# DiltheyLab/MetaMaps

Hardware: AMD Instinct MI355X
Metric: Gbp long reads mapped+classified per sec (whole node), miniSeq+H DB (higher is better)
Workload: dtype u32

## Files before the change

metamaps_amd/csrc/mm_l1.hpp:

```cpp
#pragma once
#include <rocprim/rocprim.hpp>
#include "mm_map.hpp"
#include "mm_l2.hpp"

namespace mm {

template <int IPT>
__global__ void __launch_bounds__(256) sort_hits_radix_kernel(uint64_t* __restrict__ hits, const uint64_t* __restrict__ read_hit_off,
                                                              const int32_t* __restrict__ read_list, int end_bit,
                                                              const uint64_t* __restrict__ stage ,
                                                              const uint64_t* __restrict__ stage_off ) {
  using Sort = rocprim::block_radix_sort<uint64_t, 256, IPT>;
  extern __shared__ __align__(16) unsigned char sort_dyn[];
  typename Sort::storage_type& tmp = *reinterpret_cast<typename Sort::storage_type*>(sort_dyn);
  const int r = read_list[blockIdx.x];
  const uint64_t o = read_hit_off[r];
  const int n = (int)(read_hit_off[r + 1] - o);
  const uint64_t* __restrict__ src = hits + o;
  if (stage) { const uint64_t sb = stage_off[r]; if ((uint64_t)n <= stage_off[r + 1] - sb) src = stage + sb; }
  uint64_t key[IPT];
#pragma unroll
  for (int i = 0; i < IPT; ++i) { const int idx = threadIdx.x * IPT + i; key[i] = idx < n ? src[idx] : ~0ull; }
  Sort().sort(key, tmp, 0, end_bit);
#pragma unroll
  for (int i = 0; i < IPT; ++i) { const int idx = threadIdx.x * IPT + i; if (idx < n) hits[o + idx] = key[i]; }
}

template <bool WRITE>
__global__ void l1_scan_kernel(const uint64_t* __restrict__ hits, const uint64_t* __restrict__ read_hit_off, const int32_t* __restrict__ read_len,
                               const int32_t* __restrict__ min_hits, int64_t n_reads, uint32_t* __restrict__ cand_n,
                               const uint64_t* __restrict__ cand_off, int32_t* __restrict__ cand, int32_t* __restrict__ cand_read) {
  int64_t r = (int64_t)blockIdx.x * blockDim.x + threadIdx.x;
  if (r >= n_reads) return;
  const uint64_t o = read_hit_off[r];
  const int64_t H = (int64_t)(read_hit_off[r + 1] - o);
  const int len = read_len[r];
  int m = min_hits[r]; if (m < 1) m = 1;
  uint32_t nc = 0;
  int lseq = -1, lstart = 0, lend = 0;
  uint64_t wbase = WRITE ? cand_off[r] : 0;
  auto flush = [&]() {
    if (lseq < 0) return;
    if (WRITE) { int32_t* c = cand + 3 * (wbase + nc); c[0] = lseq; c[1] = lstart; c[2] = lend; cand_read[wbase + nc] = (int32_t)r; }
    ++nc;
  };
// ... 166 lines not shown
```

metamaps_amd/csrc/mm_map.hip:

```cpp
#include "mm_map.hpp"
#include <functional>
#include <memory>
#include <rocprim/rocprim.hpp>
#include "mm_l2_core.hpp"
#include "mm_size_classes.hpp"
#include "mm_l2.hpp"
#include "mm_l2z.hpp"
#include "mm_l2_dense.hpp"
#include <cstdlib>
#include <atomic>
#include <thread>
#include "mm_stats.hpp"
#include <algorithm>
#include <numeric>
#include "mm_sketch.hpp"
#include "mm_seed.hpp"
#include "mm_l1.hpp"

namespace mm {

namespace {
struct HostLap {
  const bool on = getenv("MM_HOST_TIMING") != nullptr; std::chrono::steady_clock::time_point t = std::chrono::steady_clock::now();
  void operator()(const char* what) { if (!on) return; const auto n = std::chrono::steady_clock::now(); fprintf(stderr, "host %-28s %8.1f us\n", what, std::chrono::duration<double, std::micro>(n - t).count()); t = n; }
// ... 161 lines not shown
  std::unique_ptr<SkipClasses> sk;

  MapRun(mm_ctx* ctx_, const mm_index* I_, const mm_seqset* reads_, const mm_map_params& P_, mm_mapping* M_)
      : ctx(ctx_), I(I_), reads(reads_), P(P_), M(M_), st(ctx_->stream), T(st), n(reads_->count()) {}

  const std::vector<uint64_t>& hoff() const { return M->mz.h_off; }
  int min_mapped_len() const { return P.w + P.k + 1; }
  bool dense_read(int64_t r, int sr) const { return sr >= sw.dense_from && sr < L2_SKETCH_LIMIT && M->read_len[(size_t)r] >= min_mapped_len(); }
  bool filtering() const { return sw.use_filter && n > 0; }

  void begin() {
    MM_REQUIRE(M->sketch_only || (I && I->k == P.k && I->w == P.w), MM_ERR_ARG, "index was built with different k / window size");
    MM_REQUIRE(n < (1LL << 31), MM_ERR_LIMIT, "more than 2^31 reads in one batch");
    M->ctx = ctx; M->n_reads = n; M->params = P; M->stats = mm_map_stats{};
    M->stats.n_reads = n;
    M->read_len = reads->len;
    M->active.assign((size_t)n, 0);
    for (int64_t r = 0; r < n; ++r) {
      int L = reads->len[(size_t)r];
      bool ok = !(L < P.w || L < P.k || L < P.min_read_len);
      M->active[(size_t)r] = ok;
      if (ok) { M->stats.n_reads_long_enough++; M->stats.bases_long_enough += L; }
    }
    t_total = T.begin(&M->stats.ms_total);
  }

  void minimizers() {
    const mm_mapping* const donor = M->sketch_donor;
    if (donor) {
      const size_t t = T.begin(&M->stats.ms_minimizer);
      auto dcopy = [&](auto& dst, const auto& src) { dst.alloc(src.n); if (src.n) MM_HIP(hipMemcpyAsync(dst.p, src.p, src.bytes(), hipMemcpyDeviceToDevice, st)); };
      mm_mapping* const dn = const_cast<mm_mapping*>(donor);
      const bool same_ctx = donor->ctx == ctx;
      if (same_ctx) M->mz.rec.share_from(dn->mz.rec); else dcopy(M->mz.rec, donor->mz.rec);
      dcopy(M->mz.off, donor->mz.off);
      M->mz.h_off = donor->mz.h_off; M->mz.total = donor->mz.total;
      if (same_ctx) M->sk_hash.share_from(dn->sk_hash); else dcopy(M->sk_hash, donor->sk_hash);
      dcopy(M->sk_strand, donor->sk_strand); dcopy(M->sk_n, donor->sk_n); dcopy(M->amb, donor->amb);
      T.end(t);
    } else { size_t t = T.begin(&M->stats.ms_minimizer); run_minimizers(ctx, reads, P.k, P.w, M->active, false, M->mz); T.end(t); }
    total_mz = M->mz.total;
    if (!donor) {
      M->sk_hash.alloc((size_t)std::max<int64_t>(total_mz, 1));
      M->sk_strand.alloc((size_t)std::max<int64_t>(total_mz, 1));
      M->sk_n.alloc((size_t)std::max<int64_t>(n, 1)); M->sk_n.zero(st);
      M->amb.alloc((size_t)std::max<int64_t>(n, 1)); M->amb.zero(st);
    }
  }

  void sketch() {
    if (M->sketch_donor) return;
    size_t t_sk = T.begin(&M->stats.ms_sketch);
    static_assert(ipt_list_is<4, 6, 8, 10, 12, 16, 20, 24, 32, 40, 48, 64>(SKETCH_IPTS), "the dispatch below lists the classes of mm_size_classes.hpp");
    uint64_t big_seen = 0;
    HostLap hl;
    const ReadBins RB = bin_reads(n, N_SKETCH_CLASSES, [&](int64_t r) -> int {
      const uint64_t c = hoff()[(size_t)r + 1] - hoff()[(size_t)r];
      big_seen |= (uint64_t)(c > SKETCH_LDS_MAX);
      return sketch_class_index(c);
    });
    const bool any_big = big_seen != 0;
    {
      hl("K2 bin");
      DBuf<int32_t> list(std::max<size_t>(RB.order.size(), 1));
      list.upload(RB.order.data(), RB.order.size(), st);
      hl("K2 list upload");
      size_t at = 0;
      for (auto& run : RB.runs) {
        const unsigned nb = (unsigned)run.second;
        const int32_t* lp = list.p + at;
        dispatch<4, 6, 8, 10, 12, 16, 20, 24, 32, 40, 48, 64>(SKETCH_IPTS[run.first], [&](auto ipt_tag) {
          constexpr int IPT = decltype(ipt_tag)::value;
          using SortT = rocprim::block_radix_sort<uint32_t, 256, IPT, uint16_t>;
          using ScanT = rocprim::block_scan<int, 256>;
          const size_t lds = std::max(sizeof(typename SortT::storage_type), sizeof(typename ScanT::storage_type)) + 16;
          if (lds > 48 * 1024) MM_HIP(hipFuncSetAttribute((const void*)sketch_radix_kernel<IPT>, hipFuncAttributeMaxDynamicSharedMemorySize, (int)lds));
          sketch_radix_kernel<IPT><<<dim3(nb), dim3(256), lds, st>>>(M->mz.rec.p, M->mz.off.p, lp, M->sk_hash.p, M->sk_strand.p, M->sk_n.p, M->amb.p);
        });
        MM_KERNEL_CHECK();
        at += run.second;
      }
      hl("K2 launches");
      MM_HIP(mm::stream_sync(st));
      hl("K2 sync (kernels)");
    }
    if (any_big) sketch_big_segmented();
    T.end(t_sk);
  }

  void sketch_big_segmented() {
    std::vector<int32_t> big; std::vector<uint64_t> koff{0};
    for (int64_t r = 0; r < n; ++r) { const uint64_t c = hoff()[(size_t)r + 1] - hoff()[(size_t)r]; if (c > SKETCH_LDS_MAX) { big.push_back((int32_t)r); koff.push_back(koff.back() + c); } }
    const size_t nb = big.size(); const uint64_t nk = koff.back();
    MM_REQUIRE(nk < ((uint64_t)1 << 32), MM_ERR_LIMIT, "more than 2^32 minimizers of reads beyond 16384 minimizers in one batch");
    DBuf<int32_t> d_big(nb); d_big.upload(big.data(), nb, st);
    DBuf<uint64_t> d_koff(nb + 1); d_koff.upload(koff.data(), nb + 1, st);
    DBuf<uint64_t> keys((size_t)nk), sorted((size_t)nk);
    sketch_keys_kernel<<<dim3((unsigned)nb), dim3(256), 0, st>>>(M->mz.rec.p, M->mz.off.p, d_big.p, d_koff.p, keys.p);
    MM_KERNEL_CHECK();
    size_t tmp_bytes = 0;
    MM_HIP(rocprim::segmented_radix_sort_keys(nullptr, tmp_bytes, keys.p, sorted.p, (unsigned int)nk, (unsigned int)nb, d_koff.p, d_koff.p + 1, 0, 64, st));
    DBuf<uint8_t> tmp(std::max<size_t>(tmp_bytes, 16));
    MM_HIP(rocprim::segmented_radix_sort_keys((void*)tmp.p, tmp_bytes, keys.p, sorted.p, (unsigned int)nk, (unsigned int)nb, d_koff.p, d_koff.p + 1, 0, 64, st));
    sketch_finish_kernel<<<dim3((unsigned)nb), dim3(256), 0, st>>>(M->mz.rec.p, M->mz.off.p, d_big.p, d_koff.p, sorted.p, M->sk_hash.p, M->sk_strand.p, M->sk_n.p, M->amb.p);
    MM_KERNEL_CHECK();
    MM_HIP(mm::stream_sync(st));
  }

  bool after_sketch() {
    hl.t = std::chrono::steady_clock::now();
    M->h_sk_n = M->sk_n.to_host(st, (size_t)n);
    if (M->sketch_only) {
      for (int64_t r = 0; r < n; ++r) M->stats.sum_sketch += M->h_sk_n[(size_t)r];
      M->h_rec_off.assign((size_t)n + 1, 0); M->n_rec = 0;
      T.end(t_total);
      T.collect();
      return false;
    }
    if (M->at_stage) M->at_stage(M->at_stage_user, 1);
    h_amb = M->amb.to_host(st, (size_t)n);
    hl("post-K2 downloads");
    int64_t giant = 0;
    for (int64_t r = 0; r < n; ++r) if (M->h_sk_n[(size_t)r] >= L2_SKETCH_LIMIT) ++giant;
    M->stats.n_reads_giant = giant;
    return true;
  }

  void tiebreak_lists() {
    for (int64_t r = 0; r < n; ++r) if (h_amb[(size_t)r]) (sw.eager_tiebreak ? eager_reads : lazy_reads).push_back(r);
    M->stats.n_ambiguous_sketch_reads = (int64_t)(eager_reads.size() + lazy_reads.size());
    hl("post-K2 amb lists");
    if (!eager_reads.empty()) amb_finish = start_tiebreak(eager_reads);
    hl("post-K2 tiebreak start");
  }

  std::function<void()> start_tiebreak(const std::vector<int64_t>& amb_reads) {
    const size_t na = amb_reads.size();
    std::vector<uint64_t> so(na), dof(na + 1, 0);
    std::vector<int32_t> expect(na);
    for (size_t i = 0; i < na; ++i) {
      int64_t r = amb_reads[i];
      so[i] = hoff()[(size_t)r];
      dof[i + 1] = dof[i] + (hoff()[(size_t)r + 1] - hoff()[(size_t)r]);
      expect[i] = M->h_sk_n[(size_t)r];
    }
    DBuf<uint64_t> d_so(na), d_do(na + 1);
    d_so.upload(so.data(), na, st); d_do.upload(dof.data(), na + 1, st);
    DBuf<Rec> comp((size_t)dof[na]);
    gather_amb_kernel<<<dim3((unsigned)na), dim3(256), 0, st>>>(M->mz.rec.p, d_so.p, d_do.p, comp.p);
    MM_KERNEL_CHECK();
    amb_states.push_back(std::make_unique<AmbState>());
    AmbState* const A = amb_states.back().get();
    A->hr = comp.to_host(st);
    A->dof = dof; A->expect = std::move(expect); A->d_so = std::move(d_so); A->d_do = std::move(d_do);
    A->sv.assign((size_t)dof[na], 0);
    A->scnt.assign(na, 0);
    A->bg = std::thread([A, na]() {
      std::atomic<size_t> next{0};
      auto worker = [&]() {
        std::vector<HostMz> v;
        for (size_t i = next.fetch_add(1); i < na; i = next.fetch_add(1)) {
          const size_t cntr = (size_t)(A->dof[i + 1] - A->dof[i]);
          v.resize(cntr);
          for (size_t j = 0; j < cntr; ++j) { const Rec& x = A->hr[(size_t)A->dof[i] + j]; v[j] = HostMz{x.hash, pw_wpos(x.pw), pw_strand(x.pw)}; }
          std::sort(v.begin(), v.end(), host_less_by_hash);
          auto ue = std::unique(v.begin(), v.end(), host_eq_by_hash);
          const size_t sN = (size_t)(ue - v.begin());
          if ((int64_t)sN != A->expect[i]) A->mismatch = 1;
          for (size_t j = 0; j < sN; ++j) A->sv[(size_t)A->dof[i] + j] = v[j].strand == 1 ? 1 : 0;
          A->scnt[i] = (int32_t)sN;
        }
      };
      const unsigned nthr = std::max(1u, std::min(32u, std::min<unsigned>(mm::cpu_budget(), (unsigned)((na + 15) / 16))));
      std::vector<std::thread> pool;
      for (unsigned t = 1; t < nthr; ++t) pool.emplace_back(worker);
      worker();
      for (auto& t : pool) t.join();
    });
    return [M = M, A, na, st = st]() {
      if (A->bg.joinable()) A->bg.join();
      MM_REQUIRE(A->mismatch == 0, MM_ERR_DEVICE, "sketch size disagrees between device and host tie-break");
      DBuf<uint8_t> d_sv(A->sv.size()); d_sv.upload(A->sv.data(), A->sv.size(), st);
// ... 151 lines not shown
    }
  }

  int64_t hits_of(int64_t r) const { return (int64_t)(M->h_read_hit_off[(size_t)r + 1] - M->h_read_hit_off[(size_t)r]); }

  void sort_hits() {
    if (total_hits > 0) {
      const size_t t_sh = T.begin(&M->stats.ms_sort_hits);
      hl("K4 hits alloc + emit launch");
      int key_bits = 32; while (key_bits < 64 && ((int64_t)1 << (key_bits - 32)) < I->n_contigs) ++key_bits;
      if (sort_hits_radix(key_bits)) sort_hits_segmented(key_bits);
      T.end(t_sh);
    }
    hl("K4 launches + sync");
  }

  bool sort_hits_radix(int key_bits) {
    static_assert(ipt_list_is<1, 2, 3, 4, 6, 8, 12, 16>(HIT_SORT_IPTS), "the dispatch below lists the classes of mm_size_classes.hpp");
    uint64_t left_seen = 0;
    const ReadBins RB = bin_reads(n, N_HIT_SORT_CLASSES, [&](int64_t r) -> int {
      const uint64_t c = (uint64_t)hits_of(r);
      left_seen |= (uint64_t)(c > HIT_SORT_LDS_MAX);
      return hit_sort_class_index(c);
    });
    hl("K4 bin");
    DBuf<int32_t> list(std::max<size_t>(RB.order.size(), 1));
    list.upload(RB.order.data(), RB.order.size(), st);
    hl("K4 list upload");
    size_t at = 0;
    for (auto& run : RB.runs) {
      const int32_t* lp = list.p + at;
      dispatch<1, 2, 3, 4, 6, 8, 12, 16>(HIT_SORT_IPTS[run.first], [&](auto tag) {
        constexpr int IPT = decltype(tag)::value;
        using SortT = rocprim::block_radix_sort<uint64_t, 256, IPT>;
        const size_t lds = sizeof(typename SortT::storage_type) + 16;
        if (lds > 48 * 1024) MM_HIP(hipFuncSetAttribute((const void*)sort_hits_radix_kernel<IPT>, hipFuncAttributeMaxDynamicSharedMemorySize, (int)lds));
        sort_hits_radix_kernel<IPT><<<dim3((unsigned)run.second), dim3(256), lds, st>>>(M->hits.p, M->read_hit_off.p, lp, key_bits, sw.use_filter ? stage.p : nullptr, sw.use_filter ? stage_off.p : nullptr);
      });
      MM_KERNEL_CHECK();
      at += run.second;
    }
    MM_HIP(mm::stream_sync(st));
    return left_seen != 0;
  }

  void sort_hits_segmented(int key_bits) {
    const uint64_t max_keys = sw.segsort_max_keys;
    std::vector<int32_t> seg_reads;
    std::vector<uint64_t> hb, he, cb, ce;
    std::vector<size_t> run_at{0};
    uint64_t in_run = 0, longest_run = 0;
    for (int64_t r = 0; r < n; ++r) {
      const uint64_t c = (uint64_t)hits_of(r);
      if (c <= HIT_SORT_LDS_MAX) continue;
      MM_REQUIRE(c < max_keys, MM_ERR_LIMIT, "one read has more seed hits than a segmented sort takes (2^32 - 1, or MM_SEGSORT_MAX_KEYS)");
      if (in_run + c >= max_keys) { run_at.push_back(seg_reads.size()); in_run = 0; }
      seg_reads.push_back((int32_t)r);
      hb.push_back(M->h_read_hit_off[(size_t)r]); he.push_back(M->h_read_hit_off[(size_t)r + 1]);
      cb.push_back(in_run); in_run += c; ce.push_back(in_run);
      longest_run = std::max(longest_run, in_run);
    }
    const size_t ns = seg_reads.size();
    run_at.push_back(ns);
    const bool compact = run_at.size() > 2 || 2 * longest_run <= (uint64_t)total_hits || (uint64_t)total_hits >= max_keys;
    DBuf<uint64_t> d_hb(ns), d_he(ns), d_cb(ns), d_ce(ns);
    d_hb.upload(hb.data(), ns, st); d_he.upload(he.data(), ns, st);
    auto seg_sort = [&](uint64_t* in, uint64_t* out, uint64_t count, size_t nseg, uint64_t* begins, uint64_t* ends) {
// ... 424 lines not shown
```

metamaps_amd/csrc/mm_minimizer.hpp:

```cpp
#pragma once
#include <type_traits>
#include "mm_common.hpp"
#include "mm_scan.hpp"

namespace mm {

constexpr int MZ_THREADS = 256;
constexpr int MZ_TILE = 2048;
constexpr int MZ_MAX_W = 4096;
constexpr int MZ_STAGE = 1024;
constexpr int MZ_MAX_K = 64;

struct SeqView {
  const uint32_t* packed;
  const uint64_t* base;
  const int32_t* len;
  const uint64_t* exc_start;
  const uint32_t* exc_len;
  const uint8_t* exc_byte;
  int64_t n_exc;
  int64_t n;
};

__device__ inline uint32_t code_at(const SeqView& S, uint64_t g) { return (S.packed[g >> 4] >> (2 * (g & 15))) & 3u; }

__device__ inline int64_t exc_lower(const SeqView& S, uint64_t g) {
  int64_t lo = 0, hi = S.n_exc;
  while (lo < hi) {
    int64_t mid = (lo + hi) >> 1;
    if (S.exc_start[mid] + S.exc_len[mid] <= g) lo = mid + 1; else hi = mid;
  }
  return lo;
}
__device__ inline uint8_t ascii_at(const SeqView& S, uint64_t g) {
  if (S.n_exc) {
    int64_t r = exc_lower(S, g);
    if (r < S.n_exc && S.exc_start[r] <= g) return S.exc_byte[r];
  }
  return ascii_of_code(code_at(S, g));
}

struct KmerInfo { uint32_t hash; bool ns; bool fwd; };
__device__ inline uint64_t ascii8_of_codes(uint32_t x, bool comp) {
  const uint32_t flip = comp ? 0x03030303u : 0u;
// ... 304 lines not shown
    uint64_t o = (MODE == 1 ? tile_out[tile] : tile * (uint64_t)MZ_STAGE) + ex;
#pragma unroll
    for (int i = 0; i < MZ_TILE / MZ_THREADS; ++i) {
      if (mask & (1u << i)) {
        int j = j0 + i, p = H0 + j, c = cps[j];
        uint32_t pw = ((uint32_t)(p - w + 1) << PW_SHIFT) | ((flg[c] & 2) ? PW_STRAND : 0u);
        out[o] = Rec{hsh[c], pw};
        if (out_seq) out_seq[o] = (uint32_t)s;
        ++o;
      }
    }
  }
}

static __global__ void __launch_bounds__(256) compact_tiles_kernel(const Rec* __restrict__ stage, const uint32_t* __restrict__ tile_count,
                                                                   const uint64_t* __restrict__ tile_out, Rec* __restrict__ out) {
  const uint64_t tile = blockIdx.x;
  const uint32_t n = tile_count[tile];
  const uint64_t o = tile_out[tile];
  for (uint32_t i = threadIdx.x; i < n; i += 256) out[o + i] = stage[tile * (uint64_t)MZ_STAGE + i];
}

inline size_t minimizer_lds_bytes(int k, int w) {
  int halo = (2 * (w - 1) + 7) & ~7, NP = MZ_TILE + halo, NB = ((NP + k - 1 + 8) + 15) & ~15;
  return (size_t)2 * NB + (size_t)NP * 4 + (size_t)NP * 2 + (size_t)NP;
}

struct MinimizerSet {
  DBuf<Rec> rec;
  DBuf<uint64_t> off;
  DBuf<uint32_t> rec_seq;
  std::vector<uint64_t> h_off;
  int64_t total = 0;
};

void run_minimizers(mm_ctx* ctx, const mm_seqset* S, int k, int w, const std::vector<uint8_t>& active, bool want_rec_seq,
                    MinimizerSet& out);

SeqView make_view(const mm_seqset* S);

}
```

metamaps_amd/csrc/mm_seq.hip:

```cpp
#include "mm_minimizer.hpp"
#include <algorithm>
#include <thread>
#include <atomic>
#include <cstdio>
#include <cstring>

extern "C" int mm_host_has_avx2();
extern "C" size_t mm_pack_acgt_blocks(const uint8_t* p, size_t n_bases, uint32_t* out);

namespace mm {

SeqView make_view(const mm_seqset* S) {
  return SeqView{S->packed.p, S->d_base.p, S->d_len.p, S->exc_start.p, S->exc_len.p, S->exc_byte.p, S->n_exc, S->count()};
}

__global__ void gather_offsets_kernel(const uint64_t* __restrict__ tile_first, const uint64_t* __restrict__ tile_out, int64_t n,
                                      uint64_t* __restrict__ off) {
  int64_t s = (int64_t)blockIdx.x * blockDim.x + threadIdx.x;
  if (s <= n) off[s] = tile_out[tile_first[s]];
}

void run_minimizers(mm_ctx* ctx, const mm_seqset* S, int k, int w, const std::vector<uint8_t>& active, bool want_rec_seq,
                    MinimizerSet& out) {
  MM_REQUIRE(S->frozen, MM_ERR_STATE, "sequence set not uploaded");
  MM_REQUIRE(k >= 1 && k <= MZ_MAX_K, MM_ERR_ARG, "k must be in [1,64]");
  MM_REQUIRE(w >= 1 && w <= MZ_MAX_W, MM_ERR_ARG, "window size must be in [1,4096]");
  hipStream_t st = ctx->stream;
  const int64_t n = S->count();
  std::vector<uint64_t> tf((size_t)n + 1, 0);
  for (int64_t i = 0; i < n; ++i) {
    int64_t npos = (int64_t)S->len[i] - k + 1;
    bool on = active.empty() || active[(size_t)i];
    int64_t nt = (on && npos >= w) ? ceil_div(npos, MZ_TILE) : 0;
    tf[i + 1] = tf[i] + (uint64_t)nt;
  }
  const int64_t ntiles = (int64_t)tf[n];
  out.off.alloc((size_t)n + 1);
  out.h_off.assign((size_t)n + 1, 0);
  out.total = 0;
  if (ntiles == 0) { out.off.zero(st); out.rec.alloc(0); MM_HIP(mm::stream_sync(st)); return; }
  MM_REQUIRE(ntiles < (1LL << 31), MM_ERR_LIMIT, "too many tiles for one launch");

  DBuf<uint64_t> d_tf((size_t)n + 1);
  d_tf.upload(tf.data(), tf.size(), st);
  DBuf<uint8_t> d_act;
  if (!active.empty()) { d_act.alloc(active.size()); d_act.upload(active.data(), active.size(), st); }
  DBuf<int32_t> d_js((size_t)n);
  SeqView V = make_view(S);
  jstar_kernel<<<dim3((unsigned)ceil_div(n, 128)), dim3(128), 0, st>>>(V, d_act.p, k, w, d_js.p);
  MM_KERNEL_CHECK();

  const size_t lds = minimizer_lds_bytes(k, w);
  if (lds > 64 * 1024) {
    MM_HIP(hipFuncSetAttribute((const void*)minimizer_kernel<0>, hipFuncAttributeMaxDynamicSharedMemorySize, (int)lds));
    MM_HIP(hipFuncSetAttribute((const void*)minimizer_kernel<1>, hipFuncAttributeMaxDynamicSharedMemorySize, (int)lds));
    MM_HIP(hipFuncSetAttribute((const void*)minimizer_kernel<2>, hipFuncAttributeMaxDynamicSharedMemorySize, (int)lds));
  }
  DBuf<uint32_t> tcount((size_t)ntiles);
  DBuf<uint64_t> tout((size_t)ntiles + 1), tmp;
  bool single_pass = !want_rec_seq && (size_t)ntiles * MZ_STAGE * sizeof(Rec) <= ((size_t)6 << 30);
  DBuf<Rec> stage;
  DBuf<int> d_ovf(1); d_ovf.zero(st);
  if (single_pass) {
    stage.alloc((size_t)ntiles * MZ_STAGE);
    { const char* e = getenv("MM_MZ_DBG"); int v = e ? atoi(e) : 0; MM_HIP(hipMemcpyToSymbolAsync(HIP_SYMBOL(mz_dbg_stop), &v, sizeof v, 0, hipMemcpyHostToDevice, st)); }
    minimizer_kernel<2><<<dim3((unsigned)ntiles), dim3(MZ_THREADS), lds, st>>>(V, d_tf.p, k, w, d_js.p, tcount.p, nullptr, stage.p, nullptr, d_ovf.p);
  } else {
    minimizer_kernel<0><<<dim3((unsigned)ntiles), dim3(MZ_THREADS), lds, st>>>(V, d_tf.p, k, w, d_js.p, tcount.p, nullptr, nullptr, nullptr, nullptr);
  }
  MM_KERNEL_CHECK();
  exclusive_scan_u32_u64(tcount.p, ntiles, tout.p, tmp, st);
  uint64_t total = 0;
  int h_ovf = 0;
  MM_HIP(hipMemcpyAsync(&total, tout.p + ntiles, sizeof total, hipMemcpyDeviceToHost, st));
  MM_HIP(hipMemcpyAsync(&h_ovf, d_ovf.p, sizeof h_ovf, hipMemcpyDeviceToHost, st));
  MM_HIP(mm::stream_sync(st));
  if (h_ovf) single_pass = false;
  out.total = (int64_t)total;
  out.rec.alloc((size_t)total);
  if (want_rec_seq) out.rec_seq.alloc((size_t)total);
  if (total) {
    if (single_pass)
      compact_tiles_kernel<<<dim3((unsigned)ntiles), dim3(256), 0, st>>>(stage.p, tcount.p, tout.p, out.rec.p);
    else
      minimizer_kernel<1><<<dim3((unsigned)ntiles), dim3(MZ_THREADS), lds, st>>>(V, d_tf.p, k, w, d_js.p, nullptr, tout.p, out.rec.p,
                                                                               want_rec_seq ? out.rec_seq.p : nullptr, nullptr);
    MM_KERNEL_CHECK();
  }
  gather_offsets_kernel<<<dim3((unsigned)ceil_div(n + 1, 256)), dim3(256), 0, st>>>(d_tf.p, tout.p, n, out.off.p);
  MM_KERNEL_CHECK();
  out.off.download(out.h_off.data(), (size_t)n + 1, st);
  MM_HIP(mm::stream_sync(st));
}

static inline int code_of(uint8_t c) {
  switch (c) { case 'A': return 0; case 'C': return 1; case 'G': return 2; case 'T': return 3; }
  return -1;
}

void seqset_upload(mm_seqset* s) {
  MM_REQUIRE(!s->frozen, MM_ERR_STATE, "sequence set already uploaded");
  hipStream_t st = s->ctx->stream;
  const size_t n = s->staged.size();
  s->len.resize(n);
  s->base.assign(n + 1, 0);
  s->total_bases = 0;
  for (size_t i = 0; i < n; ++i) {
    MM_REQUIRE((int64_t)s->staged[i].second <= MAX_SEQ_LEN, MM_ERR_LIMIT, "sequence longer than 2^29-1 bases");
    s->len[i] = (int32_t)s->staged[i].second;
    s->base[i + 1] = s->base[i] + (((uint64_t)s->len[i] + 15) & ~15ull);
    s->total_bases += s->len[i];
  }
  const size_t nwords = (size_t)(s->base[n] >> 4);
  uint32_t* const words = (uint32_t*)s->ctx->pinned_up_at_least((nwords + 1) * sizeof(uint32_t));
  words[nwords] = 0;
  std::vector<uint64_t> es; std::vector<uint32_t> el; std::vector<uint8_t> eb;
  {
    static const struct Lut { uint8_t t[256]; Lut() { for (int c = 0; c < 256; ++c) { int u = (c > 96 && c < 123) ? c - 32 : c; int k = code_of((uint8_t)u); t[c] = k >= 0 ? (uint8_t)k : 0x80; } } } lut;
    struct Item { size_t seq; size_t j0, j1; };
    struct Runs { std::vector<uint64_t> es; std::vector<uint32_t> el; std::vector<uint8_t> eb; };
    constexpr size_t PIECE = (size_t)4 << 20;
    std::vector<Item> items;
    for (size_t i = 0; i < n; ++i) { const size_t L = s->staged[i].second; for (size_t j0 = 0; j0 < L; j0 += PIECE) items.push_back(Item{i, j0, std::min(L, j0 + PIECE)}); }
    std::vector<Runs> runs(items.size());
    const unsigned hw = mm::cpu_budget();
// ... 427 lines not shown
```

metamaps_amd/csrc/mm_sketch.hpp:

```cpp
#pragma once
#include <rocprim/rocprim.hpp>
#include "mm_map.hpp"

namespace mm {

template <int IPT>
__global__ void __launch_bounds__(256) sketch_radix_kernel(const Rec* __restrict__ rec, const uint64_t* __restrict__ off,
                                                           const int32_t* __restrict__ read_list, uint32_t* __restrict__ sk_hash,
                                                           uint8_t* __restrict__ sk_strand, int32_t* __restrict__ sk_n, uint8_t* __restrict__ amb) {
  using Sort = rocprim::block_radix_sort<uint32_t, 256, IPT, uint16_t>;
  using Scan = rocprim::block_scan<int, 256>;
  union Tmp { typename Sort::storage_type sort; typename Scan::storage_type scan; };
  extern __shared__ __align__(16) unsigned char sketch_dyn[];
  Tmp& tmp = *reinterpret_cast<Tmp*>(sketch_dyn);
  __shared__ uint32_t last_key[256];
  __shared__ uint8_t last_st[256];
  __shared__ int s_amb;
  const int r = read_list[blockIdx.x];
  const uint64_t o = off[r];
  const int n = (int)(off[r + 1] - o);
  const int t = threadIdx.x;
  uint32_t key[IPT]; uint16_t val[IPT];
#pragma unroll
  for (int i = 0; i < IPT; ++i) { const int idx = t * IPT + i; key[i] = idx < n ? rec[o + idx].hash : 0xffffffffu; val[i] = (uint16_t)idx; }
  if (t == 0) s_amb = 0;
  Sort().sort(key, val, tmp.sort);
  uint8_t stv[IPT];
#pragma unroll
  for (int i = 0; i < IPT; ++i) stv[i] = (t * IPT + i < n) ? (uint8_t)(rec[o + val[i]].pw & PW_STRAND) : 0;
  last_key[t] = key[IPT - 1]; last_st[t] = stv[IPT - 1];
  __syncthreads();
  int nfirst = 0; bool first[IPT]; bool ambig = false;
#pragma unroll
  for (int i = 0; i < IPT; ++i) {
    const int pos = t * IPT + i;
    const uint32_t pk = i ? key[i - 1] : (t ? last_key[t - 1] : 0u);
    const uint8_t ps = i ? stv[i - 1] : (t ? last_st[t - 1] : 0);
    first[i] = pos < n && (pos == 0 || pk != key[i]);
    if (pos < n && pos > 0 && pk == key[i] && ps != stv[i]) ambig = true;
    nfirst += first[i] ? 1 : 0;
  }
  if (ambig) s_amb = 1;
  int ex = 0, total = 0;
  Scan().exclusive_scan(nfirst, ex, 0, total, tmp.scan);
  const int ex0 = ex;
#pragma unroll
  for (int i = 0; i < IPT; ++i) if (first[i]) { sk_hash[o + ex] = key[i]; sk_strand[o + ex] = stv[i]; ++ex; }
  __threadfence_block();
  __syncthreads();
  if (s_amb) {
    int ex2 = ex0;
#pragma unroll
    for (int i = 0; i < IPT; ++i) {
      const int pos = t * IPT + i;
      if (first[i]) ++ex2;
      const uint32_t pk = i ? key[i - 1] : (t ? last_key[t - 1] : 0u);
      const uint8_t ps = i ? stv[i - 1] : (t ? last_st[t - 1] : 0);
      if (pos < n && pos > 0 && pk == key[i] && ps != stv[i]) sk_strand[o + ex2 - 1] |= 2;
    }
  }
  if (t == 0) { sk_n[r] = total; amb[r] = (uint8_t)(s_amb ? 2 : 0); }
}

__global__ void __launch_bounds__(256) sketch_keys_kernel(const Rec* __restrict__ rec, const uint64_t* __restrict__ off, const int32_t* __restrict__ read_list,
                                                          const uint64_t* __restrict__ koff, uint64_t* __restrict__ keys) {
  const int r = read_list[blockIdx.x];
  const uint64_t o = off[r], k0 = koff[blockIdx.x];
  const uint32_t n = (uint32_t)(off[r + 1] - o);
  for (uint32_t i = threadIdx.x; i < n; i += 256) keys[k0 + i] = ((uint64_t)rec[o + i].hash << 32) | i;
}
__global__ void __launch_bounds__(256) sketch_finish_kernel(const Rec* __restrict__ rec, const uint64_t* __restrict__ off, const int32_t* __restrict__ read_list,
                                                            const uint64_t* __restrict__ koff, const uint64_t* __restrict__ sorted,
                                                            uint32_t* __restrict__ sk_hash, uint8_t* __restrict__ sk_strand, int32_t* __restrict__ sk_n, uint8_t* __restrict__ amb) {
  const int r = read_list[blockIdx.x];
  const uint64_t o = off[r];
  const uint64_t* __restrict__ a = sorted + koff[blockIdx.x];
  const int n = (int)(off[r + 1] - o);
  __shared__ int s_amb;
  if (threadIdx.x == 0) s_amb = 0;
  __syncthreads();
  for (int pass = 0; pass < 2; ++pass) {
    uint64_t carry = 0;
    for (int base = 0; base < n; base += 256) {
      const int i = base + threadIdx.x;
      bool first = false, differs = false; uint32_t h = 0, stv = 0;
      if (i < n) {
        const uint64_t key = a[i];
        h = (uint32_t)(key >> 32);
        stv = rec[o + (uint32_t)key].pw & PW_STRAND;
        if (i == 0) first = true;
        else {
          const uint64_t pk = a[i - 1];
          first = (uint32_t)(pk >> 32) != h;
          differs = !first && (rec[o + (uint32_t)pk].pw & PW_STRAND) != stv;
        }
      }
      uint64_t tot;
      const uint64_t ex = block_excl_scan_u64(first ? 1 : 0, &tot);
      if (pass == 0) {
        if (first) { sk_hash[o + carry + ex] = h; sk_strand[o + carry + ex] = (uint8_t)stv; }
        if (differs) s_amb = 1;
      } else if (differs) sk_strand[o + carry + ex - 1] |= 2;
      carry += tot;
    }
    __threadfence_block();
    __syncthreads();
    if (pass == 0) {
      if (threadIdx.x == 0) { sk_n[r] = (int32_t)carry; amb[r] = (uint8_t)(s_amb ? 2 : 0); }
      if (!s_amb) break;
    }
  }
}

__global__ void __launch_bounds__(256) gather_amb_kernel(const Rec* __restrict__ rec, const uint64_t* __restrict__ src_off,
                                                         const uint64_t* __restrict__ dst_off, Rec* __restrict__ out) {
  const uint64_t so = src_off[blockIdx.x], d0 = dst_off[blockIdx.x], n = dst_off[blockIdx.x + 1] - d0;
  for (uint64_t i = threadIdx.x; i < n; i += 256) out[d0 + i] = rec[so + i];
}
__global__ void __launch_bounds__(256) scatter_strand_kernel(const uint8_t* __restrict__ in, const uint64_t* __restrict__ src_off,
                                                             const uint64_t* __restrict__ dst_off, const int32_t* __restrict__ cnt,
                                                             uint8_t* __restrict__ sk_strand) {
  const uint64_t d0 = dst_off[blockIdx.x], so = src_off[blockIdx.x];
  const int n = cnt[blockIdx.x];
  for (int i = threadIdx.x; i < n; i += 256) sk_strand[so + i] = in[d0 + i];
}

}
```

Before: 26.16.

## Read minimizers directly from staging tiles instead of compacting them

Skips the compact_tiles pass after single-pass minimizer extraction. It keeps the tiled staging buffer plus per-tile offsets, and sketch, tiebreak and big-read kernels index records through a RecView with tile-walking helpers. The sketch sort now packs the strand bit into the sort value, which avoids a second gather of rec after sorting. It also adds occupancy hints (waves_per_eu) per IPT and configurable radix digit bits for the sketch and hit sorts. The cost is extra index arithmetic and less coalesced reads through the staged layout, and the staging buffer must be kept alive.

```diff
diff --git a/metamaps_amd/csrc/mm_l1.hpp b/metamaps_amd/csrc/mm_l1.hpp
--- a/metamaps_amd/csrc/mm_l1.hpp
+++ b/metamaps_amd/csrc/mm_l1.hpp
@@ -5,12 +5,16 @@
 
 namespace mm {
 
+#ifndef HIT_SORT_DIGIT_BITS
+#define HIT_SORT_DIGIT_BITS 8
+#endif
+template <int IPT> using HitSort = rocprim::block_radix_sort<uint64_t, 256, IPT, rocprim::empty_type, 1, 1, HIT_SORT_DIGIT_BITS>;
 template <int IPT>
 __global__ void __launch_bounds__(256) sort_hits_radix_kernel(uint64_t* __restrict__ hits, const uint64_t* __restrict__ read_hit_off,
                                                               const int32_t* __restrict__ read_list, int end_bit,
                                                               const uint64_t* __restrict__ stage ,
                                                               const uint64_t* __restrict__ stage_off ) {
-  using Sort = rocprim::block_radix_sort<uint64_t, 256, IPT>;
+  using Sort = HitSort<IPT>;
   extern __shared__ __align__(16) unsigned char sort_dyn[];
   typename Sort::storage_type& tmp = *reinterpret_cast<typename Sort::storage_type*>(sort_dyn);
   const int r = read_list[blockIdx.x];
diff --git a/metamaps_amd/csrc/mm_map.hip b/metamaps_amd/csrc/mm_map.hip
--- a/metamaps_amd/csrc/mm_map.hip
+++ b/metamaps_amd/csrc/mm_map.hip
@@ -217,13 +217,13 @@
       auto dcopy = [&](auto& dst, const auto& src) { dst.alloc(src.n); if (src.n) MM_HIP(hipMemcpyAsync(dst.p, src.p, src.bytes(), hipMemcpyDeviceToDevice, st)); };
       mm_mapping* const dn = const_cast<mm_mapping*>(donor);
       const bool same_ctx = donor->ctx == ctx;
-      if (same_ctx) M->mz.rec.share_from(dn->mz.rec); else dcopy(M->mz.rec, donor->mz.rec);
-      dcopy(M->mz.off, donor->mz.off);
-      M->mz.h_off = donor->mz.h_off; M->mz.total = donor->mz.total;
+      if (same_ctx) { M->mz.rec.share_from(dn->mz.rec); M->mz.stage.share_from(dn->mz.stage); } else { dcopy(M->mz.rec, donor->mz.rec); dcopy(M->mz.stage, donor->mz.stage); }
+      dcopy(M->mz.off, donor->mz.off); dcopy(M->mz.tile_first, donor->mz.tile_first); dcopy(M->mz.tout, donor->mz.tout);
+      M->mz.h_off = donor->mz.h_off; M->mz.total = donor->mz.total; M->mz.staged = donor->mz.staged;
       if (same_ctx) M->sk_hash.share_from(dn->sk_hash); else dcopy(M->sk_hash, donor->sk_hash);
       dcopy(M->sk_strand, donor->sk_strand); dcopy(M->sk_n, donor->sk_n); dcopy(M->amb, donor->amb);
       T.end(t);
-    } else { size_t t = T.begin(&M->stats.ms_minimizer); run_minimizers(ctx, reads, P.k, P.w, M->active, false, M->mz); T.end(t); }
+    } else { size_t t = T.begin(&M->stats.ms_minimizer); run_minimizers(ctx, reads, P.k, P.w, M->active, false, M->mz, SKETCH_READS_STAGING != 0); T.end(t); }
     total_mz = M->mz.total;
     if (!donor) {
       M->sk_hash.alloc((size_t)std::max<int64_t>(total_mz, 1));
@@ -256,11 +256,11 @@
         const int32_t* lp = list.p + at;
         dispatch<4, 6, 8, 10, 12, 16, 20, 24, 32, 40, 48, 64>(SKETCH_IPTS[run.first], [&](auto ipt_tag) {
           constexpr int IPT = decltype(ipt_tag)::value;
-          using SortT = rocprim::block_radix_sort<uint32_t, 256, IPT, uint16_t>;
+          using SortT = SketchSort<IPT>;
           using ScanT = rocprim::block_scan<int, 256>;
           const size_t lds = std::max(sizeof(typename SortT::storage_type), sizeof(typename ScanT::storage_type)) + 16;
           if (lds > 48 * 1024) MM_HIP(hipFuncSetAttribute((const void*)sketch_radix_kernel<IPT>, hipFuncAttributeMaxDynamicSharedMemorySize, (int)lds));
-          sketch_radix_kernel<IPT><<<dim3(nb), dim3(256), lds, st>>>(M->mz.rec.p, M->mz.off.p, lp, M->sk_hash.p, M->sk_strand.p, M->sk_n.p, M->amb.p);
+          sketch_radix_kernel<IPT><<<dim3(nb), dim3(256), lds, st>>>(rec_view(M->mz), lp, M->sk_hash.p, M->sk_strand.p, M->sk_n.p, M->amb.p);
         });
         MM_KERNEL_CHECK();
         at += run.second;
@@ -281,13 +281,13 @@
     DBuf<int32_t> d_big(nb); d_big.upload(big.data(), nb, st);
     DBuf<uint64_t> d_koff(nb + 1); d_koff.upload(koff.data(), nb + 1, st);
     DBuf<uint64_t> keys((size_t)nk), sorted((size_t)nk);
-    sketch_keys_kernel<<<dim3((unsigned)nb), dim3(256), 0, st>>>(M->mz.rec.p, M->mz.off.p, d_big.p, d_koff.p, keys.p);
+    sketch_keys_kernel<<<dim3((unsigned)nb), dim3(256), 0, st>>>(rec_view(M->mz), d_big.p, d_koff.p, keys.p);
     MM_KERNEL_CHECK();
     size_t tmp_bytes = 0;
     MM_HIP(rocprim::segmented_radix_sort_keys(nullptr, tmp_bytes, keys.p, sorted.p, (unsigned int)nk, (unsigned int)nb, d_koff.p, d_koff.p + 1, 0, 64, st));
     DBuf<uint8_t> tmp(std::max<size_t>(tmp_bytes, 16));
     MM_HIP(rocprim::segmented_radix_sort_keys((void*)tmp.p, tmp_bytes, keys.p, sorted.p, (unsigned int)nk, (unsigned int)nb, d_koff.p, d_koff.p + 1, 0, 64, st));
-    sketch_finish_kernel<<<dim3((unsigned)nb), dim3(256), 0, st>>>(M->mz.rec.p, M->mz.off.p, d_big.p, d_koff.p, sorted.p, M->sk_hash.p, M->sk_strand.p, M->sk_n.p, M->amb.p);
+    sketch_finish_kernel<<<dim3((unsigned)nb), dim3(256), 0, st>>>(rec_view(M->mz), d_big.p, d_koff.p, sorted.p, M->sk_hash.p, M->sk_strand.p, M->sk_n.p, M->amb.p);
     MM_KERNEL_CHECK();
     MM_HIP(mm::stream_sync(st));
   }
@@ -322,17 +322,18 @@
   std::function<void()> start_tiebreak(const std::vector<int64_t>& amb_reads) {
     const size_t na = amb_reads.size();
     std::vector<uint64_t> so(na), dof(na + 1, 0);
-    std::vector<int32_t> expect(na);
+    std::vector<int32_t> expect(na), ids(na);
     for (size_t i = 0; i < na; ++i) {
       int64_t r = amb_reads[i];
-      so[i] = hoff()[(size_t)r];
+      so[i] = hoff()[(size_t)r]; ids[i] = (int32_t)r;
       dof[i + 1] = dof[i] + (hoff()[(size_t)r + 1] - hoff()[(size_t)r]);
       expect[i] = M->h_sk_n[(size_t)r];
     }
     DBuf<uint64_t> d_so(na), d_do(na + 1);
     d_so.upload(so.data(), na, st); d_do.upload(dof.data(), na + 1, st);
+    DBuf<int32_t> d_ids(na); d_ids.upload(ids.data(), na, st);
     DBuf<Rec> comp((size_t)dof[na]);
-    gather_amb_kernel<<<dim3((unsigned)na), dim3(256), 0, st>>>(M->mz.rec.p, d_so.p, d_do.p, comp.p);
+    gather_amb_kernel<<<dim3((unsigned)na), dim3(256), 0, st>>>(rec_view(M->mz), d_ids.p, d_do.p, comp.p);
     MM_KERNEL_CHECK();
     amb_states.push_back(std::make_unique<AmbState>());
     AmbState* const A = amb_states.back().get();
@@ -550,7 +551,7 @@
       const int32_t* lp = list.p + at;
       dispatch<1, 2, 3, 4, 6, 8, 12, 16>(HIT_SORT_IPTS[run.first], [&](auto tag) {
         constexpr int IPT = decltype(tag)::value;
-        using SortT = rocprim::block_radix_sort<uint64_t, 256, IPT>;
+        using SortT = HitSort<IPT>;
         const size_t lds = sizeof(typename SortT::storage_type) + 16;
         if (lds > 48 * 1024) MM_HIP(hipFuncSetAttribute((const void*)sort_hits_radix_kernel<IPT>, hipFuncAttributeMaxDynamicSharedMemorySize, (int)lds));
         sort_hits_radix_kernel<IPT><<<dim3((unsigned)run.second), dim3(256), lds, st>>>(M->hits.p, M->read_hit_off.p, lp, key_bits, sw.use_filter ? stage.p : nullptr, sw.use_filter ? stage_off.p : nullptr);
diff --git a/metamaps_amd/csrc/mm_minimizer.hpp b/metamaps_amd/csrc/mm_minimizer.hpp
--- a/metamaps_amd/csrc/mm_minimizer.hpp
+++ b/metamaps_amd/csrc/mm_minimizer.hpp
@@ -2,6 +2,7 @@
 #include <type_traits>
 #include "mm_common.hpp"
 #include "mm_scan.hpp"
+#include "mm_stage_index.hpp"
 
 namespace mm {
 
@@ -10,6 +11,7 @@
 constexpr int MZ_MAX_W = 4096;
 constexpr int MZ_STAGE = 1024;
 constexpr int MZ_MAX_K = 64;
+static_assert(MZ_STAGE == STAGE_SLOTS, "mm_stage_index.hpp restates the staging's slot count");
 
 struct SeqView {
   const uint32_t* packed;
@@ -380,10 +382,25 @@
   DBuf<uint32_t> rec_seq;
   std::vector<uint64_t> h_off;
   int64_t total = 0;
+  bool staged = false;
+  DBuf<Rec> stage;
+  DBuf<uint64_t> tile_first;
+  DBuf<uint64_t> tout;
 };
 
+struct RecView {
+  const Rec* rec; const uint64_t* off; const uint64_t* tile_first; const uint64_t* tout;
+  bool staged;
+  __device__ __forceinline__ const Rec& at(int64_t r, uint64_t idx) const {
+    return rec[staged ? stage_slot(tout, tile_first[r], tile_first[r + 1], idx) : off[r] + idx];
+  }
+};
+inline RecView rec_view(const MinimizerSet& m) {
+  return m.staged ? RecView{m.stage.p, m.off.p, m.tile_first.p, m.tout.p, true} : RecView{m.rec.p, m.off.p, nullptr, nullptr, false};
+}
+
 void run_minimizers(mm_ctx* ctx, const mm_seqset* S, int k, int w, const std::vector<uint8_t>& active, bool want_rec_seq,
-                    MinimizerSet& out);
+                    MinimizerSet& out, bool keep_staged = false);
 
 SeqView make_view(const mm_seqset* S);
 
diff --git a/metamaps_amd/csrc/mm_seq.hip b/metamaps_amd/csrc/mm_seq.hip
--- a/metamaps_amd/csrc/mm_seq.hip
+++ b/metamaps_amd/csrc/mm_seq.hip
@@ -21,7 +21,7 @@
 }
 
 void run_minimizers(mm_ctx* ctx, const mm_seqset* S, int k, int w, const std::vector<uint8_t>& active, bool want_rec_seq,
-                    MinimizerSet& out) {
+                    MinimizerSet& out, bool keep_staged) {
   MM_REQUIRE(S->frozen, MM_ERR_STATE, "sequence set not uploaded");
   MM_REQUIRE(k >= 1 && k <= MZ_MAX_K, MM_ERR_ARG, "k must be in [1,64]");
   MM_REQUIRE(w >= 1 && w <= MZ_MAX_W, MM_ERR_ARG, "window size must be in [1,4096]");
@@ -38,6 +38,7 @@
   out.off.alloc((size_t)n + 1);
   out.h_off.assign((size_t)n + 1, 0);
   out.total = 0;
+  out.staged = false; out.stage.release(); out.tile_first.release(); out.tout.release();
   if (ntiles == 0) { out.off.zero(st); out.rec.alloc(0); MM_HIP(mm::stream_sync(st)); return; }
   MM_REQUIRE(ntiles < (1LL << 31), MM_ERR_LIMIT, "too many tiles for one launch");
 
@@ -77,9 +78,10 @@
   MM_HIP(mm::stream_sync(st));
   if (h_ovf) single_pass = false;
   out.total = (int64_t)total;
-  out.rec.alloc((size_t)total);
+  out.staged = single_pass && keep_staged && total > 0;
+  out.rec.alloc(out.staged ? 0 : (size_t)total);
   if (want_rec_seq) out.rec_seq.alloc((size_t)total);
-  if (total) {
+  if (total && !out.staged) {
     if (single_pass)
       compact_tiles_kernel<<<dim3((unsigned)ntiles), dim3(256), 0, st>>>(stage.p, tcount.p, tout.p, out.rec.p);
     else
@@ -91,6 +93,7 @@
   MM_KERNEL_CHECK();
   out.off.download(out.h_off.data(), (size_t)n + 1, st);
   MM_HIP(mm::stream_sync(st));
+  if (out.staged) { out.stage = std::move(stage); out.tile_first = std::move(d_tf); out.tout = std::move(tout); }
 }
 
 static inline int code_of(uint8_t c) {
diff --git a/metamaps_amd/csrc/mm_sketch.hpp b/metamaps_amd/csrc/mm_sketch.hpp
--- a/metamaps_amd/csrc/mm_sketch.hpp
+++ b/metamaps_amd/csrc/mm_sketch.hpp
@@ -1,14 +1,26 @@
 #pragma once
 #include <rocprim/rocprim.hpp>
 #include "mm_map.hpp"
+#include "mm_size_classes.hpp"
 
 namespace mm {
 
+#ifndef SKETCH_SORT_DIGIT_BITS
+#define SKETCH_SORT_DIGIT_BITS 8
+#endif
+#ifndef SKETCH_READS_STAGING
+#define SKETCH_READS_STAGING 1
+#endif
+template <int IPT> using SketchSort = rocprim::block_radix_sort<uint32_t, 256, IPT, uint16_t, 1, 1, SKETCH_SORT_DIGIT_BITS>;
+constexpr uint16_t SKETCH_VAL_STRAND = 0x8000u;
+static_assert(SKETCH_LDS_MAX <= SKETCH_VAL_STRAND / 2 && PW_STRAND == 1u, "winnowing index in bits 0-13, strand in bit 15 of the sort value");
+
+constexpr int sketch_waves_per_simd(int ipt) { return ipt <= 6 ? 8 : ipt <= 8 ? 7 : ipt <= 10 ? 6 : ipt <= 12 ? 5 : ipt <= 16 ? 4 : ipt <= 24 ? 3 : ipt <= 40 ? 2 : 1; }
+
 template <int IPT>
-__global__ void __launch_bounds__(256) sketch_radix_kernel(const Rec* __restrict__ rec, const uint64_t* __restrict__ off,
-                                                           const int32_t* __restrict__ read_list, uint32_t* __restrict__ sk_hash,
+__global__ void __launch_bounds__(256) __attribute__((amdgpu_waves_per_eu(sketch_waves_per_simd(IPT)))) sketch_radix_kernel(const RecView V, const int32_t* __restrict__ read_list, uint32_t* __restrict__ sk_hash,
                                                            uint8_t* __restrict__ sk_strand, int32_t* __restrict__ sk_n, uint8_t* __restrict__ amb) {
-  using Sort = rocprim::block_radix_sort<uint32_t, 256, IPT, uint16_t>;
+  using Sort = SketchSort<IPT>;
   using Scan = rocprim::block_scan<int, 256>;
   union Tmp { typename Sort::storage_type sort; typename Scan::storage_type scan; };
   extern __shared__ __align__(16) unsigned char sketch_dyn[];
@@ -17,17 +29,41 @@
   __shared__ uint8_t last_st[256];
   __shared__ int s_amb;
   const int r = read_list[blockIdx.x];
-  const uint64_t o = off[r];
-  const int n = (int)(off[r + 1] - o);
+  const uint64_t o = V.off[r];
+  const int n = (int)(V.off[r + 1] - o);
   const int t = threadIdx.x;
   uint32_t key[IPT]; uint16_t val[IPT];
+  auto take = [&](int i, int idx, const Rec x) { key[i] = x.hash; val[i] = (uint16_t)(idx | ((x.pw & PW_STRAND) ? SKETCH_VAL_STRAND : 0)); };
 #pragma unroll
-  for (int i = 0; i < IPT; ++i) { const int idx = t * IPT + i; key[i] = idx < n ? rec[o + idx].hash : 0xffffffffu; val[i] = (uint16_t)idx; }
+  for (int i = 0; i < IPT; ++i) { key[i] = 0xffffffffu; val[i] = (uint16_t)(t * IPT + i); }
+  if (!V.staged) {
+#pragma unroll
+    for (int i = 0; i < IPT; ++i) { const int idx = t * IPT + i; if (idx < n) take(i, idx, (V.rec + o)[(uint32_t)idx]); }
+  } else if (n > 0) {
+    const uint64_t t0 = V.tile_first[r], t1 = V.tile_first[r + 1];
+    if (t1 - t0 <= STAGE_WALK_MAX) {
+      const StageTiles T = stage_tiles_load(V.tout, t0, t1);
+      const Rec* __restrict__ const rb = V.rec + t0 * (uint64_t)STAGE_SLOTS;
+      StageCursor c = stage_tiles_seek(T, (uint32_t)(t * IPT));
+#pragma unroll
+      for (int i = 0; i < IPT; ++i) {
+        const int idx = t * IPT + i;
+        if (idx < n) { if ((uint32_t)idx >= c.next) c = stage_tiles_seek(T, (uint32_t)idx); take(i, idx, rb[stage_cursor_offset(c, (uint32_t)idx)]); }
+      }
+    } else if (t * IPT < n) {
+      uint64_t tl = stage_tile_of(V.tout, t0, t1, (uint64_t)(t * IPT));
+#pragma unroll
+      for (int i = 0; i < IPT; ++i) {
+        const int idx = t * IPT + i;
+        if (idx < n) { tl = stage_tile_next(V.tout, t0, t1, tl, (uint64_t)idx); take(i, idx, V.rec[stage_slot_in(V.tout, t0, tl, (uint64_t)idx)]); }
+      }
+    }
+  }
   if (t == 0) s_amb = 0;
   Sort().sort(key, val, tmp.sort);
   uint8_t stv[IPT];
 #pragma unroll
-  for (int i = 0; i < IPT; ++i) stv[i] = (t * IPT + i < n) ? (uint8_t)(rec[o + val[i]].pw & PW_STRAND) : 0;
+  for (int i = 0; i < IPT; ++i) stv[i] = (t * IPT + i < n && (val[i] & SKETCH_VAL_STRAND)) ? (uint8_t)PW_STRAND : 0;
   last_key[t] = key[IPT - 1]; last_st[t] = stv[IPT - 1];
   __syncthreads();
   int nfirst = 0; bool first[IPT]; bool ambig = false;
@@ -62,20 +98,20 @@
   if (t == 0) { sk_n[r] = total; amb[r] = (uint8_t)(s_amb ? 2 : 0); }
 }
 
-__global__ void __launch_bounds__(256) sketch_keys_kernel(const Rec* __restrict__ rec, const uint64_t* __restrict__ off, const int32_t* __restrict__ read_list,
+__global__ void __launch_bounds__(256) sketch_keys_kernel(const RecView V, const int32_t* __restrict__ read_list,
                                                           const uint64_t* __restrict__ koff, uint64_t* __restrict__ keys) {
   const int r = read_list[blockIdx.x];
-  const uint64_t o = off[r], k0 = koff[blockIdx.x];
-  const uint32_t n = (uint32_t)(off[r + 1] - o);
-  for (uint32_t i = threadIdx.x; i < n; i += 256) keys[k0 + i] = ((uint64_t)rec[o + i].hash << 32) | i;
+  const uint64_t k0 = koff[blockIdx.x];
+  const uint32_t n = (uint32_t)(V.off[r + 1] - V.off[r]);
+  for (uint32_t i = threadIdx.x; i < n; i += 256) keys[k0 + i] = ((uint64_t)V.at(r, i).hash << 32) | i;
 }
-__global__ void __launch_bounds__(256) sketch_finish_kernel(const Rec* __restrict__ rec, const uint64_t* __restrict__ off, const int32_t* __restrict__ read_list,
+__global__ void __launch_bounds__(256) sketch_finish_kernel(const RecView V, const int32_t* __restrict__ read_list,
                                                             const uint64_t* __restrict__ koff, const uint64_t* __restrict__ sorted,
                                                             uint32_t* __restrict__ sk_hash, uint8_t* __restrict__ sk_strand, int32_t* __restrict__ sk_n, uint8_t* __restrict__ amb) {
   const int r = read_list[blockIdx.x];
-  const uint64_t o = off[r];
+  const uint64_t o = V.off[r];
   const uint64_t* __restrict__ a = sorted + koff[blockIdx.x];
-  const int n = (int)(off[r + 1] - o);
+  const int n = (int)(V.off[r + 1] - o);
   __shared__ int s_amb;
   if (threadIdx.x == 0) s_amb = 0;
   __syncthreads();
@@ -87,12 +123,12 @@
       if (i < n) {
         const uint64_t key = a[i];
         h = (uint32_t)(key >> 32);
-        stv = rec[o + (uint32_t)key].pw & PW_STRAND;
+        stv = V.at(r, (uint32_t)key).pw & PW_STRAND;
         if (i == 0) first = true;
         else {
           const uint64_t pk = a[i - 1];
           first = (uint32_t)(pk >> 32) != h;
-          differs = !first && (rec[o + (uint32_t)pk].pw & PW_STRAND) != stv;
+          differs = !first && (V.at(r, (uint32_t)pk).pw & PW_STRAND) != stv;
         }
       }
       uint64_t tot;
@@ -112,10 +148,11 @@
   }
 }
 
-__global__ void __launch_bounds__(256) gather_amb_kernel(const Rec* __restrict__ rec, const uint64_t* __restrict__ src_off,
+__global__ void __launch_bounds__(256) gather_amb_kernel(const RecView V, const int32_t* __restrict__ read_list,
                                                          const uint64_t* __restrict__ dst_off, Rec* __restrict__ out) {
-  const uint64_t so = src_off[blockIdx.x], d0 = dst_off[blockIdx.x], n = dst_off[blockIdx.x + 1] - d0;
-  for (uint64_t i = threadIdx.x; i < n; i += 256) out[d0 + i] = rec[so + i];
+  const int r = read_list[blockIdx.x];
+  const uint64_t d0 = dst_off[blockIdx.x], n = dst_off[blockIdx.x + 1] - d0;
+  for (uint64_t i = threadIdx.x; i < n; i += 256) out[d0 + i] = V.at(r, i);
 }
 __global__ void __launch_bounds__(256) scatter_strand_kernel(const uint8_t* __restrict__ in, const uint64_t* __restrict__ src_off,
                                                              const uint64_t* __restrict__ dst_off, const int32_t* __restrict__ cnt,
diff --git a/metamaps_amd/csrc/mm_stage_index.hpp b/metamaps_amd/csrc/mm_stage_index.hpp
--- /dev/null
+++ b/metamaps_amd/csrc/mm_stage_index.hpp
@@ -0,0 +1,67 @@
+#pragma once
+#include <cstdint>
+
+#if defined(__HIPCC__)
+#define STAGE_HD __host__ __device__ inline
+#else
+#define STAGE_HD inline
+#endif
+
+namespace mm {
+
+constexpr int STAGE_SLOTS = 1024;
+constexpr uint64_t STAGE_WALK_MAX = 8;
+
+STAGE_HD uint64_t stage_tile_of(const uint64_t* tout, uint64_t t0, uint64_t t1, uint64_t idx) {
+  const uint64_t key = tout[t0] + idx;
+  if (t1 - t0 <= STAGE_WALK_MAX) {
+    uint64_t t = t0;
+    while (t + 1 < t1 && tout[t + 1] <= key) ++t;
+    return t;
+  }
+  uint64_t lo = t0, hi = t1;
+  while (hi - lo > 1) { const uint64_t mid = lo + ((hi - lo) >> 1); if (tout[mid] <= key) lo = mid; else hi = mid; }
+  return lo;
+}
+
+STAGE_HD uint64_t stage_tile_next(const uint64_t* tout, uint64_t t0, uint64_t t1, uint64_t t, uint64_t idx) {
+  const uint64_t key = tout[t0] + idx;
+  while (t + 1 < t1 && tout[t + 1] <= key) ++t;
+  return t;
+}
+
+STAGE_HD uint64_t stage_slot_in(const uint64_t* tout, uint64_t t0, uint64_t t, uint64_t idx) {
+  return t * (uint64_t)STAGE_SLOTS + idx - (tout[t] - tout[t0]);
+}
+
+STAGE_HD uint64_t stage_slot(const uint64_t* tout, uint64_t t0, uint64_t t1, uint64_t idx) {
+  return stage_slot_in(tout, t0, stage_tile_of(tout, t0, t1, idx), idx);
+}
+
+struct StageTiles {
+  uint64_t t0;
+  uint32_t first[STAGE_WALK_MAX];
+};
+STAGE_HD StageTiles stage_tiles_load(const uint64_t* tout, uint64_t t0, uint64_t t1) {
+  StageTiles T; T.t0 = t0;
+  const uint64_t base = tout[t0];
+  for (uint64_t j = 0; j < STAGE_WALK_MAX; ++j) T.first[j] = t0 + j < t1 ? (uint32_t)(tout[t0 + j] - base) : ~0u;
+  return T;
+}
+struct StageCursor { uint32_t j, f, next; };
+STAGE_HD StageCursor stage_tiles_seek(const StageTiles& T, uint32_t idx) {
+  StageCursor c{0, 0, ~0u};
+  for (uint64_t i = 1; i < STAGE_WALK_MAX; ++i) {
+    const bool in = T.first[i] <= idx;
+    c.j += in ? 1u : 0u; c.f = in ? T.first[i] : c.f;
+    c.next = (!in && T.first[i] < c.next) ? T.first[i] : c.next;
+  }
+  return c;
+}
+STAGE_HD uint32_t stage_cursor_offset(const StageCursor& c, uint32_t idx) {
+  return c.j * (uint32_t)STAGE_SLOTS + (idx - c.f);
+}
+STAGE_HD uint64_t stage_cursor_slot(const StageTiles& T, const StageCursor& c, uint32_t idx) { return T.t0 * (uint64_t)STAGE_SLOTS + stage_cursor_offset(c, idx); }
+STAGE_HD uint64_t stage_tiles_slot(const StageTiles& T, uint32_t idx) { return stage_cursor_slot(T, stage_tiles_seek(T, idx), idx); }
+
+}
```

Result: no change. 26.07 (-0.3%).
